# arpitbansal297/Cold-Diffusion-Models

Hardware: AMD Instinct MI355X
Metric: unet_train_imgs_per_sec (higher is better)
Workload: dtype f32 storage/accumulate; dense-conv GEMM operands bf16x3; 1 GPU; CelebA-128 denoising cold diffusion (BASELINE config 3): Unet(dim=64,(1,2,4,8),ch=3) @128x128, T=200, optimizer step = 2 micro-batches x 32 img (one fused forward / backward pass over all of them: same draws, same gradient sum) + Adam + EMA/10; per_gpu_batch=32, gradient_accumulate_every=2, parallelism=single

## Files before the change

cold-diffusion-models_amd/csrc/cdf_epilogue.h:

```cpp
#pragma once
#include "cdf_common.h"

static inline int cdf_epi_vec_ok(int Cout, const float* y, int ldy, const float* bias, const float* sbias, int ld_sbias, const float* res,
                                 int ldr, const float* pre, int ldp, const float* mul, int ldm) {
    const uintptr_t ptrs = (uintptr_t)y | (uintptr_t)bias | (uintptr_t)sbias | (uintptr_t)res | (uintptr_t)pre | (uintptr_t)mul;
    const int pitches = ldy | (sbias ? ld_sbias : 0) | (res ? ldr : 0) | (pre ? ldp : 0) | (mul ? ldm : 0);
    return (Cout % 4 == 0 && (ptrs & 15) == 0 && (pitches & 3) == 0) ? 1 : 0;
}

__device__ __forceinline__ void cdf_ld4(float* v, const float* p, int n, bool vec) {
    if (vec) {
        const float4 t = *(const float4*)p;
        v[0] = t.x; v[1] = t.y; v[2] = t.z; v[3] = t.w;
    } else {
#pragma unroll
        for (int e = 0; e < 4; ++e) v[e] = e < n ? p[e] : 0.f;
    }
}

__device__ __forceinline__ void cdf_st4(float* p, const float* v, int n, bool vec) {
    if (vec) {
        *(float4*)p = make_float4(v[0], v[1], v[2], v[3]);
    } else {
#pragma unroll
        for (int e = 0; e < 4; ++e)
            if (e < n) p[e] = v[e];
    }
}

template <int BN, int RP, int NTHR = 256, class Args, class Phase, class RowMap>
__device__ __forceinline__ void cdf_epilogue_rows(const Args& a, const Phase& ph, float* Y, const float* cs, int m_base, int n_base, int M,
                                                  int tid, RowMap rowmap, long long pix_off = 0) {
    constexpr int CP = BN + 8, TPR = BN / 4, RPS = NTHR / TPR;
    const int c4 = (tid % TPR) * 4, co = n_base + c4;
    if (co >= a.Cout) return;
    const int nval = a.Cout - co < 4 ? a.Cout - co : 4;
    const bool vec = a.vec != 0;
    const bool direct = (a.os == 1 && a.QH == a.OH && a.QW == a.OW);
    const int qhw = a.QH * a.QW;
    float bv[4] = {0.f, 0.f, 0.f, 0.f};
    if (a.bias) cdf_ld4(bv, a.bias + co, nval, vec);
    long long prev = 0, o_pre = co, o_mul = co, o_res = co, o_y = co, o_ys = co;
    bool first = true;
    for (int p = tid / TPR; p < RP; p += RPS) {
        const int m = m_base + rowmap(p);
        if (m >= M) continue;
        long long opix;
        int b;
        if (direct) {
            opix = m;
            b = m / qhw;
        } else {
            const int qx = m % a.QW, t2 = m / a.QW;
            const int qy = t2 % a.QH;
            b = t2 / a.QH;
            opix = ((long long)b * a.OH + qy * a.os + ph.oy) * a.OW + qx * a.os + ph.ox;
        }
        opix += pix_off;
        if (first) {
            o_pre += opix * a.ldp; o_mul += opix * a.ldm; o_res += opix * a.ldr; o_y += opix * a.ldy; o_ys += opix * a.ld_ys;
            first = false;
        } else {
            const int d = (int)(opix - prev);
            o_pre += (long long)d * a.ldp; o_mul += (long long)d * a.ldm; o_res += (long long)d * a.ldr; o_y += (long long)d * a.ldy;
            o_ys += (long long)d * a.ld_ys;
        }
        prev = opix;
        const float4 t = *(const float4*)(cs + p * CP + c4);
        float v[4] = {t.x + bv[0], t.y + bv[1], t.z + bv[2], t.w + bv[3]};
        float u[4];
        if (a.sbias) {
            cdf_ld4(u, a.sbias + (long long)b * a.ld_sbias + co, nval, vec);
#pragma unroll
            for (int e = 0; e < 4; ++e) v[e] += u[e];
        }
        if (a.pre && (a.io_bf & CDF_IO_PRE_GRAD)) {
            float gr[4];
#pragma unroll
            for (int e = 0; e < 4; ++e) {
                if (a.act == 1) {
                    v[e] = cdf_gelu_both(v[e], gr[e]);
                } else {
                    gr[e] = cdf_silu_grad(v[e]);
                    v[e] = cdf_silu(v[e]);
                }
            }
            if (a.io_bf & CDF_IO_PRE_BF16) cdf_st4_bf(a.pre, o_pre, gr);
            else cdf_st4(a.pre + o_pre, gr, nval, vec);
        } else {
        if (a.pre) {
            if (a.io_bf & CDF_IO_PRE_BF16) cdf_st4_bf(a.pre, o_pre, v);
            else cdf_st4(a.pre + o_pre, v, nval, vec);
        }
        if (a.act == 1) {
#pragma unroll
            for (int e = 0; e < 4; ++e) v[e] = cdf_gelu(v[e]);
        } else if (a.act == 2) {
#pragma unroll
            for (int e = 0; e < 4; ++e) v[e] = cdf_silu(v[e]);
        } else if (a.act == 3) {
#pragma unroll
            for (int e = 0; e < 4; ++e) v[e] = fmaxf(v[e], 0.0f);
        }
        }
        if (a.mul_mode) {
            if (a.io_bf & CDF_IO_MUL_BF16) cdf_ld4_bf(u, a.mul, o_mul);
            else cdf_ld4(u, a.mul + o_mul, nval, vec);
#pragma unroll
            for (int e = 0; e < 4; ++e) v[e] *= (a.mul_mode == 1 ? cdf_gelu_grad(u[e]) : (a.mul_mode == 2 ? cdf_silu_grad(u[e]) : u[e]));
        }
        if (a.res) {
            if (a.io_bf & CDF_IO_RES_BF16) cdf_ld4_bf(u, a.res, o_res);
            else cdf_ld4(u, a.res + o_res, nval, vec);
#pragma unroll
            for (int e = 0; e < 4; ++e) v[e] += u[e];
        }
        if (Y) {
            float* dst = Y + o_y;
            if (a.accumulate) {
                cdf_ld4(u, dst, nval, vec);
#pragma unroll
                for (int e = 0; e < 4; ++e) v[e] += u[e];
            }
            cdf_st4(dst, v, nval, vec);
        }
        if (a.ys_hi && vec)
            cdf_split_store4(a.ys_hi + o_ys, a.ys_lo ? a.ys_lo + o_ys : nullptr, v);
    }
}

typedef unsigned cdf_u32x2 __attribute__((ext_vector_type(2)));
#ifdef CDF_EMU
#define CDF_OPAQUE_V(x) ((void)0)
#else
#define CDF_OPAQUE_V(x) asm volatile("" : "+v"(x))
#endif

template <int ACT_, int PRE_, int MUL_, bool RES_, bool ACC_, bool HASY_, int YS_, int IO_>
struct EpiSpec {
    static constexpr int ACT = ACT_, PRE = PRE_, MUL = MUL_, YS = YS_, IO = IO_;
    static constexpr bool RES = RES_, ACC = ACC_, HASY = HASY_;
};
typedef EpiSpec<0, 0, 0, false, false, true, 0, 0> EpiPlain;
typedef EpiSpec<0, 0, 0, true, false, true, 0, 0> EpiRes;
typedef EpiSpec<1, 1, 0, false, false, false, 2, 0> EpiGeluPrePlanes;
typedef EpiSpec<1, 0, 0, false, false, false, 2, 0> EpiGeluPlanes;
typedef EpiSpec<0, 0, 1, false, false, false, 2, 0> EpiMulGeluPlanes;
typedef EpiSpec<0, 0, 0, false, true, true, 0, 0> EpiAcc;
typedef EpiSpec<0, 0, 0, false, false, false, 1, 0> EpiBfPlain;
typedef EpiSpec<0, 0, 0, true, false, false, 1, CDF_IO_RES_BF16> EpiBfRes;
typedef EpiSpec<1, 1, 0, false, false, false, 1, CDF_IO_PRE_BF16> EpiBfGeluPre;
typedef EpiSpec<1, 0, 0, false, false, false, 1, 0> EpiBfGelu;
typedef EpiSpec<0, 0, 1, false, false, false, 1, CDF_IO_MUL_BF16> EpiBfMulGelu;
#define CDF_EPI_NSPEC 11

template <class Args>
static inline int cdf_epi_select(const Args& a) {
    if (!a.vec || a.os != 1 || a.QH != a.OH || a.QW != a.OW) return 0;
    const bool pre = a.pre != nullptr, mul = a.mul_mode != 0, res = a.res != nullptr, acc = a.accumulate != 0, y = a.y != nullptr;
    const int ys = a.ys_hi ? (a.ys_lo ? 2 : 1) : 0, io = a.io_bf;
    if (io & CDF_IO_PRE_GRAD) return 0;
    auto is = [&](int ACT, int PRE, int MUL, bool RES, bool ACC, bool HASY, int YS, int IO) {
        return a.act == ACT && (pre ? 1 : 0) == PRE && a.mul_mode == MUL && res == RES && acc == ACC && y == HASY && ys == YS &&
               (io & ((PRE ? CDF_IO_PRE_BF16 : 0) | (MUL ? CDF_IO_MUL_BF16 : 0) | (RES ? CDF_IO_RES_BF16 : 0))) == IO;
    };
    (void)mul;
    if (is(0, 0, 0, false, false, true, 0, 0)) return 1;
    if (is(0, 0, 0, true, false, true, 0, 0)) return 2;
    if (is(1, 1, 0, false, false, false, 2, 0)) return 3;
    if (is(1, 0, 0, false, false, false, 2, 0)) return 4;
    if (is(0, 0, 1, false, false, false, 2, 0)) return 5;
    if (is(0, 0, 0, false, true, true, 0, 0)) return 6;
    if (is(0, 0, 0, false, false, false, 1, 0)) return 7;
    if (is(0, 0, 0, true, false, false, 1, CDF_IO_RES_BF16)) return 8;
    if (is(1, 1, 0, false, false, false, 1, CDF_IO_PRE_BF16)) return 9;
    if (is(1, 0, 0, false, false, false, 1, 0)) return 10;
    if (is(0, 0, 1, false, false, false, 1, CDF_IO_MUL_BF16)) return 11;
    return 0;
}

template <int TILE_ROWS, int BN, class Args>
__device__ __forceinline__ bool cdf_epi_tile_ok(const Args& a, int M) {
    return a.epi != 0 && M % TILE_ROWS == 0 && a.Cout % BN == 0 && (a.sbias == nullptr || (a.QH * a.QW) % TILE_ROWS == 0);
}

template <bool BF>
__device__ __forceinline__ f32x4_t cdf_ld_raw4(const void* base, unsigned off) {
    if constexpr (BF) {
        const cdf_u32x2 t = *(const cdf_u32x2*)((const unsigned short*)base + off);
        f32x4_t r = {__uint_as_float(t[0]), __uint_as_float(t[1]), 0.f, 0.f};
        return r;
    } else {
        return *(const f32x4_t*)((const float*)base + off);
    }
}
template <bool BF>
__device__ __forceinline__ f32x4_t cdf_cvt_raw4(const f32x4_t& r) {
    if constexpr (BF) {
        const unsigned x = __float_as_uint(r[0]), y = __float_as_uint(r[1]);
        f32x4_t v = {__uint_as_float(x << 16), __uint_as_float(x & 0xFFFF0000u), __uint_as_float(y << 16), __uint_as_float(y & 0xFFFF0000u)};
        return v;
    } else {
        return r;
    }
}
template <bool BF>
__device__ __forceinline__ void cdf_st_raw4(void* base, unsigned off, const f32x4_t& v) {
    if constexpr (BF) {
        cdf_u32x2 h;
        h[0] = cdf_pack2bf(v[0], v[1]);
        h[1] = cdf_pack2bf(v[2], v[3]);
        *(cdf_u32x2*)((unsigned short*)base + off) = h;
    } else {
        *(f32x4_t*)((float*)base + off) = v;
    }
}

template <int BN, int NTHR, class Args>
__device__ __forceinline__ void cdf_epi_load_bias(const Args& a, f32x4_t (&bs)[2], long long row0, int n_base, int tid) {
    int c4 = (tid % (BN / 4)) * 4;
    CDF_OPAQUE_V(c4);
    const int co = n_base + c4;
    const long long b = a.sbias ? row0 / (a.QH * a.QW) : 0;
    const float* pb = a.bias ? a.bias + co : (const float*)cdf_zero_page;
    const float* ps = a.sbias ? a.sbias + b * a.ld_sbias + co : (const float*)cdf_zero_page;
    bs[0] = *(const f32x4_t*)pb;
    bs[1] = *(const f32x4_t*)ps;
}

template <int BN, int RP, int NTHR, class S>
struct cdf_epi_fast {
    static constexpr int CP = BN + 8, TPR = BN / 4, RPS = NTHR / TPR, NR = RP / RPS;
    static_assert(NR >= 1 && NR * RPS == RP, "rows of a pass must divide among the threads");
    static_assert((S::RES ? 1 : 0) + (S::MUL ? 1 : 0) + (S::ACC ? 1 : 0) <= 1, "one loaded operand per row");
    static constexpr bool RES_BF = (S::IO & CDF_IO_RES_BF16) != 0, MUL_BF = (S::IO & CDF_IO_MUL_BF16) != 0, PRE_BF = (S::IO & CDF_IO_PRE_BF16) != 0;
    template <class Args>
    __device__ __forceinline__ static f32x4_t load_row(const Args& a, long long row0, int co, int p0, int k) {
        if constexpr (S::RES) {
            const void* base = RES_BF ? (const void*)((const unsigned short*)a.res + row0 * a.ldr) : (const void*)((const float*)a.res + row0 * a.ldr);
            return cdf_ld_raw4<RES_BF>(base, (unsigned)(p0 + k * RPS) * (unsigned)a.ldr + (unsigned)co);
        } else if constexpr (S::MUL != 0) {
            const void* base = MUL_BF ? (const void*)((const unsigned short*)a.mul + row0 * a.ldm) : (const void*)((const float*)a.mul + row0 * a.ldm);
            return cdf_ld_raw4<MUL_BF>(base, (unsigned)(p0 + k * RPS) * (unsigned)a.ldm + (unsigned)co);
        } else {
            return *(const f32x4_t*)(a.y + row0 * a.ldy + (unsigned)(p0 + k * RPS) * (unsigned)a.ldy + (unsigned)co);
        }
    }
    static constexpr bool LOADS = S::RES || S::MUL != 0 || S::ACC;
    template <class Args>
    __device__ __forceinline__ static void load(const Args& a, f32x4_t (&q)[NR], long long row0, int n_base, int tid) {
        if constexpr (LOADS) {
            int c4 = (tid % TPR) * 4, p0 = tid / TPR;
            CDF_OPAQUE_V(c4);
            CDF_OPAQUE_V(p0);
            const int co = n_base + c4;
#pragma unroll
            for (int k = 0; k < NR; ++k) q[k] = load_row(a, row0, co, p0, k);
        }
    }
    template <bool NEXT = false, class Args>
    __device__ __forceinline__ static void finish(const Args& a, f32x4_t (&q)[NR], const f32x4_t (&bs)[2], const float* cs, long long row0, int n_base, int tid,
                                                  long long next_row0 = 0) {
        int c4 = (tid % TPR) * 4, p0 = tid / TPR;
        CDF_OPAQUE_V(c4);
        CDF_OPAQUE_V(p0);
        const int co = n_base + c4;
        finish_rows<NEXT>(a, q, cs, row0, co, c4, p0, bs[0], bs[1], a.sbias != nullptr, next_row0);
    }
    template <bool NEXT, class Args>
    __device__ __forceinline__ static void finish_rows(const Args& a, f32x4_t (&q)[NR], const float* cs, long long row0, int co, int c4, int p0,
                                                       const f32x4_t& bv, const f32x4_t& sb, const bool has_sb, long long next_row0) {
        float* const ybase = S::HASY ? a.y + row0 * a.ldy : nullptr;
        void* const pbase = S::PRE ? (PRE_BF ? (void*)((unsigned short*)a.pre + row0 * a.ldp) : (void*)((float*)a.pre + row0 * a.ldp)) : nullptr;
        unsigned short* const hbase = S::YS ? a.ys_hi + row0 * a.ld_ys : nullptr;
        unsigned short* const lbase = S::YS == 2 ? a.ys_lo + row0 * a.ld_ys : nullptr;
        f32x4_t nxt = *(const f32x4_t*)(cs + (unsigned)p0 * CP + c4);
#pragma unroll
        for (int k = 0; k < NR; ++k) {
            const unsigned p = (unsigned)(p0 + k * RPS);
            f32x4_t v = nxt;
            if (k + 1 < NR) nxt = *(const f32x4_t*)(cs + (p + RPS) * CP + c4);
#pragma unroll
            for (int e = 0; e < 4; ++e) v[e] += bv[e];
            if (has_sb) {
#pragma unroll
                for (int e = 0; e < 4; ++e) v[e] += sb[e];
            }
            if constexpr (S::PRE == 1) cdf_st_raw4<PRE_BF>(pbase, p * (unsigned)a.ldp + (unsigned)co, v);
            if constexpr (S::ACT == 1) {
#pragma unroll
                for (int e = 0; e < 4; ++e) v[e] = cdf_gelu(v[e]);
            } else if constexpr (S::ACT == 2) {
#pragma unroll
                for (int e = 0; e < 4; ++e) v[e] = cdf_silu(v[e]);
            }
            if constexpr (S::MUL != 0) {
                const f32x4_t u = cdf_cvt_raw4<MUL_BF>(q[k]);
#pragma unroll
                for (int e = 0; e < 4; ++e) v[e] *= (S::MUL == 1 ? cdf_gelu_grad(u[e]) : (S::MUL == 2 ? cdf_silu_grad(u[e]) : u[e]));
            }
            if constexpr (S::RES) {
                const f32x4_t u = cdf_cvt_raw4<RES_BF>(q[k]);
#pragma unroll
                for (int e = 0; e < 4; ++e) v[e] += u[e];
            }
            if constexpr (S::ACC) {
#pragma unroll
                for (int e = 0; e < 4; ++e) v[e] += q[k][e];
            }
            if constexpr (NEXT && LOADS) q[k] = load_row(a, next_row0, co, p0, k);
            if constexpr (S::HASY) *(f32x4_t*)(ybase + p * (unsigned)a.ldy + (unsigned)co) = v;
            if constexpr (S::YS != 0) {
                uint2 h, l;
                cdf_split4(v[0], v[1], v[2], v[3], h, l);
                const unsigned o = p * (unsigned)a.ld_ys + (unsigned)co;
                *(uint2*)(hbase + o) = h;
                if constexpr (S::YS == 2) *(uint2*)(lbase + o) = l;
            }
            CDF_SCHED_FENCE();
        }
    }
};

template <bool BF_FAMILY, class F>
__device__ __forceinline__ void cdf_epi_dispatch(int id, F&& f) {
    if constexpr (!BF_FAMILY) {
        switch (id) {
            case 1: f(EpiPlain{}); break;
            case 2: f(EpiRes{}); break;
            case 3: f(EpiGeluPrePlanes{}); break;
            case 4: f(EpiGeluPlanes{}); break;
            case 5: f(EpiMulGeluPlanes{}); break;
            default: f(EpiAcc{}); break;
        }
    } else {
        switch (id) {
            case 7: f(EpiBfPlain{}); break;
            case 8: f(EpiBfRes{}); break;
            case 9: f(EpiBfGeluPre{}); break;
            case 10: f(EpiBfGelu{}); break;
            default: f(EpiBfMulGelu{}); break;
        }
    }
}
__device__ __forceinline__ bool cdf_epi_family_ok(int id, bool bf_family) { return bf_family ? (id >= 7 && id <= 11) : (id >= 1 && id <= 6); }


#define CDF_EPI_LNBWD 12
template <int BM, int BN, int NTHR, class Args, class Dump>
__device__ __forceinline__ void cdf_epi_lnbwd(const Args& a, float* cs, int tile_m, int tid, Dump&& dump) {
    constexpr int CP = BN + 8, TPR = BN / 4, RPS = NTHR / TPR, NR = BM / RPS;
    static_assert(NR >= 1 && NR * RPS == BM && (TPR & (TPR - 1)) == 0 && TPR <= 64, "rows divide among the threads; a row is a power-of-two lane group");
    int c4 = (tid % TPR) * 4, p0 = tid / TPR;
    CDF_OPAQUE_V(c4);
    CDF_OPAQUE_V(p0);
    const long long row0 = (long long)tile_m * BM;
    const f32x4_t g = *(const f32x4_t*)(a.bias + c4);
    const float* xb = a.ln_x + row0 * a.ld_lnx;
    const float* mb = a.ln_mean + row0;
    const float* rb = a.ln_rstd + row0;
    f32x4_t x[NR];
    float mean[NR], rstd[NR];
#pragma unroll
    for (int k = 0; k < NR; ++k) {
        const unsigned r = (unsigned)(p0 + k * RPS);
        x[k] = *(const f32x4_t*)(xb + r * (unsigned)a.ld_lnx + (unsigned)c4);
        mean[k] = mb[r];
        rstd[k] = rb[r];
    }
    dump();
    CDF_LDS_BARRIER();
    float* const ybase = a.y + row0 * a.ldy;
    const float inv_c = 1.0f / (float)BN;
    f32x4_t dg = {0.f, 0.f, 0.f, 0.f}, db = {0.f, 0.f, 0.f, 0.f};
    f32x4_t nxt = *(const f32x4_t*)(cs + (unsigned)p0 * CP + c4);
#pragma unroll
    for (int k = 0; k < NR; ++k) {
        const unsigned p = (unsigned)(p0 + k * RPS);
        const f32x4_t d = nxt;
        if (k + 1 < NR) nxt = *(const f32x4_t*)(cs + (p + RPS) * CP + c4);
        f32x4_t xh, gy, o;
#pragma unroll
        for (int e = 0; e < 4; ++e) {
            xh[e] = (x[k][e] - mean[k]) * rstd[k];
            dg[e] += d[e] * xh[e];
            db[e] += d[e];
            gy[e] = d[e] * g[e];
        }
        float s1 = (gy[0] + gy[1]) + (gy[2] + gy[3]);
        float s2 = (gy[0] * xh[0] + gy[1] * xh[1]) + (gy[2] * xh[2] + gy[3] * xh[3]);
        s1 = cdf_group_sum(s1, TPR) * inv_c;
        s2 = cdf_group_sum(s2, TPR) * inv_c;
#pragma unroll
        for (int e = 0; e < 4; ++e) o[e] = rstd[k] * (gy[e] - s1 - xh[e] * s2);
        *(f32x4_t*)(ybase + p * (unsigned)a.ldy + (unsigned)c4) = o;
        CDF_SCHED_FENCE();
    }
    CDF_LDS_BARRIER();
    float* red = cs;
    *(f32x4_t*)(red + ((unsigned)p0 * 2 + 0) * BN + c4) = dg;
    *(f32x4_t*)(red + ((unsigned)p0 * 2 + 1) * BN + c4) = db;
    CDF_LDS_BARRIER();
    for (int e = tid; e < 2 * BN; e += NTHR) {
        float t = 0.f;
#pragma unroll 4
        for (int r = 0; r < RPS; ++r) t += red[r * 2 * BN + e];
        a.ln_part[(long long)tile_m * 2 * BN + e] = t;
    }
}
```

cold-diffusion-models_amd/csrc/k_conv_rowhalo.hip:

```cpp
#include "cdf_conv_sp.h"

template <int W, int BN, int NS = 3, int NCH = 2, int BM = 256>
__global__ void __launch_bounds__(512, 1) conv_igemm_rowhalo_stream_kernel(SpxArgs a) {
    constexpr int WM = BM / 64, WN = 8 / WM, NW = 8, BK = 32, RE = 32, MT = BM / WM / 32, NB = 3;
    static_assert(BM == 256 && WM * WN == 8 && MT == 2, "8 waves (4 x 2) of 64-row tiles");
    static_assert(NCH % 2 == 0, "an even number of tap-row groups per tile returns the pipeline to row buffer 0");
    constexpr int EROWS = BM / 2;
    constexpr int TH = BM / W, HW2 = W + 2, RH = TH * HW2;
    constexpr int NSEG = (RH + 15) / 16, HRP = NSEG * 16;
    constexpr int TAG = (NSEG + NW - 1) / NW;
    constexpr int NT = BN / WN / 32;
    constexpr int SB = BN / 16 / NW;
    static_assert(SB * NW * 16 == BN || BN == 64, "B tile must split into 16-row segments");
    constexpr int SBI = BN == 64 ? 1 : SB;
    constexpr int PLANE_A = HRP * RE, ABUF = 2 * PLANE_A;
    constexpr int PLANE_B = BN * RE, BSTAGE = 2 * PLANE_B;
    constexpr int OFF_A1 = ABUF + 2 * BSTAGE, OFF_B2 = OFF_A1 + ABUF;
    CDF_DYN_SMEM(smem_raw);
    unsigned short* smem = (unsigned short*)smem_raw;
    float* const cs = (float*)(smem + OFF_A1);
    constexpr int CP = BN + 8;
    static_assert((size_t)OFF_A1 * 2 + (size_t)EROWS * CP * 4 <= 160 * 1024, "the staging tile must fit behind the live operand buffers");

    const int tid = threadIdx.x, lane = tid & 63, wave = __builtin_amdgcn_readfirstlane(tid >> 6);
    const int wm = wave / WN, wn = wave % WN;
    const int M = a.B * a.QH * a.QW;
    const int tiles_n = (a.Cout + BN - 1) / BN, tiles_m = M / BM, ntiles = tiles_m * tiles_n;
    const SpPhase& ph = a.ph[0];
    const int tpi = a.H / TH;

    const int srow = lane >> 2;
    const int q8 = ((lane & 3) ^ ((lane >> 4) & 3)) * 8;
    int a_seg[TAG], a_ry[TAG], a_x[TAG];
#pragma unroll
    for (int q = 0; q < TAG; ++q) {
        int g = wave + NW * q;
        if (g >= NSEG) g -= (g / NSEG) * NSEG;
        a_seg[q] = g;
        const int r = g * 16 + srow;
        a_ry[q] = r < RH ? r / HW2 : -(1 << 20);
        a_x[q] = r - (r / HW2) * HW2 - 1;
    }
    auto fetch_a = [&](int img, int y0, int c, int dy, int buf) {
        unsigned short* base = smem + (buf ? OFF_A1 : 0);
#pragma unroll
        for (int q = 0; q < TAG; ++q) {
            const int y = y0 + a_ry[q] + dy;
            const bool ok = img >= 0 && (unsigned)y < (unsigned)a.H && (unsigned)a_x[q] < (unsigned)W;
            const size_t off = ((size_t)(((ok ? img : 0) * a.H + (ok ? y : 0)) * W + (ok ? a_x[q] : 0))) * (unsigned)a.ldx + (unsigned)(c * BK + q8);
            unsigned short* seg = base + a_seg[q] * 16 * RE;
            CDF_GLDS16_K(ok ? a.x_hi + off : a.zero, seg);
            if constexpr (NS == 3) CDF_GLDS16_K(ok ? a.x_lo + off : a.zero, seg + PLANE_A);
        }
    };
    auto fetch_b = [&](int tile_n, int c, int wi, int stage) {
        unsigned short* st = smem + (stage == 2 ? OFF_B2 : ABUF + stage * BSTAGE);
#pragma unroll
        for (int p = 0; p < SBI; ++p) {
            const int seg = BN == 64 ? (wave & 3) : wave * SB + p;
            const int n = tile_n * BN + seg * 16 + srow;
            const int brow = n < a.Cout ? n : a.Cout - 1;
            const size_t woff = (size_t)((unsigned)wi * (unsigned)a.Cout + (unsigned)brow) * (unsigned)a.ldk + (unsigned)(c * BK + q8);
            CDF_GLDS16_K(a.w_hi + woff, st + seg * 16 * RE);
            if constexpr (NS == 3) CDF_GLDS16_K(a.w_lo + woff, st + PLANE_B + seg * 16 * RE);
        }
    };
    constexpr int NPL = NS == 3 ? 2 : 1;
    constexpr int PB = NPL * SBI, PAG = NPL * TAG;

    const int half = lane >> 5, l31 = lane & 31;
    int row0[MT];
#pragma unroll
    for (int i = 0; i < MT; ++i) {
        const int pix = wm * (BM / WM) + i * 32 + l31;
        const int py = pix / W, px = pix - py * W;
        row0[i] = py * HW2 + px + 1;
    }
    const bool late = a.dephase != 0 && wave >= NW / 2;

    auto tile_pos = [&](int v, int& img, int& y0, int& tn, int& tm) {
        if (v < ntiles) {
            const int tile = cdf_sp_swizzle(v, ntiles);
            tm = tile / tiles_n;
            tn = tile - tm * tiles_n;
            img = tm / tpi;
            y0 = (tm - img * tpi) * TH;
        } else {
            img = -1; y0 = 0; tn = 0; tm = 0;
        }
    };
    int img, y0, tile_n, tile_m;
    int v = blockIdx.x;
    tile_pos(v, img, y0, tile_n, tile_m);
    const bool fast_epi = cdf_epi_tile_ok<BM, BN>(a, M) && cdf_epi_family_ok(a.epi, NS == 1);
    fetch_a(img, y0, 0, ph.dy[0], 0);
    fetch_b(tile_n, 0, ph.wi[0], 0);
    fetch_b(tile_n, 0, ph.wi[1], 1);
    CDF_WAIT_DMA_LEAVE(PB);
    CDF_LDS_BARRIER();

    while (img >= 0) {
        int img_n, y0_n, tile_n_n, tile_m_n;
        tile_pos(v + gridDim.x, img_n, y0_n, tile_n_n, tile_m_n);
        f32x16_t acc[MT][NT];
#pragma unroll
        for (int i = 0; i < MT; ++i)
#pragma unroll
            for (int j = 0; j < NT; ++j)
#pragma unroll
                for (int r = 0; r < 16; ++r) acc[i][j][r] = 0.f;
        bf16x8_v ah[2][MT], al[2][MT], bh[2][NT], bl[2][NT];
        if (late) {
#pragma unroll
            for (int ks = 0; ks < 2; ++ks) {
#pragma unroll
                for (int i = 0; i < MT; ++i)
#pragma unroll
                    for (int e = 0; e < 8; ++e) { ah[ks][i][e] = 0; al[ks][i][e] = 0; }
#pragma unroll
                for (int j = 0; j < NT; ++j)
#pragma unroll
                    for (int e = 0; e < 8; ++e) { bh[ks][j][e] = 0; bl[ks][j][e] = 0; }
            }
        }
        auto mma_frags = [&]() { cdf_mma_tile<NS, MT, NT>(acc, ah, al, bh, bl); };
        int row0t[MT], l31t = l31;
#pragma unroll
        for (int i = 0; i < MT; ++i) row0t[i] = row0[i];
#ifndef CDF_EMU
#pragma unroll
        for (int i = 0; i < MT; ++i) asm volatile("" : "+v"(row0t[i]));
        asm volatile("" : "+v"(l31t));
#endif
        const int swbt = (l31t >> 2) & 3;
#pragma unroll
        for (int g = 0; g < 3; ++g) {
#pragma unroll
            for (int c = 0; c < NCH; ++c) {
#pragma unroll
                for (int i3 = 0; i3 < 3; ++i3) {
                    const int t = 3 * g + i3;
                    const int step = (g * NCH + c) * 3 + i3;
                    const int par = (g * NCH + c) & 1, rd = step % NB;
                    {
                        const int s2 = step + 2, gc2 = (s2 / 3) % (3 * NCH);
                        const bool over = s2 >= 9 * NCH;
                        const int g2 = gc2 / NCH, c2 = gc2 - g2 * NCH;
                        fetch_b(over ? tile_n_n : tile_n, c2, ph.wi[3 * g2 + s2 % 3], s2 % NB);
                    }
                    if (i3 == 0) {
                        const bool lastc = c + 1 == NCH, over = lastc && g == 2;
                        const int nc = lastc ? 0 : c + 1, ng = over ? 0 : (lastc ? g + 1 : g);
                        fetch_a(over ? img_n : img, over ? y0_n : y0, nc, ph.dy[3 * ng], par ^ 1);
                    }
                    int sa_e = par ? OFF_A1 : 0, sb_e = rd == 2 ? OFF_B2 : ABUF + rd * BSTAGE;
#ifndef CDF_EMU
                    asm volatile("" : "+s"(sa_e), "+s"(sb_e));
#endif
                    const unsigned short* sa = smem + sa_e;
                    const unsigned short* sb = smem + sb_e;
                    const int dx = ph.dx[t];
                    auto read_frags = [&]() {
#pragma unroll
                        for (int ks = 0; ks < 2; ++ks) {
#pragma unroll
                            for (int i = 0; i < MT; ++i) {
                                const int row = row0t[i] + dx;
                                const int off = row * RE + ((ks * 2 + half) ^ ((row >> 2) & 3)) * 8;
                                ah[ks][i] = *(const bf16x8_v*)(sa + off);
                                if constexpr (NS == 3) al[ks][i] = *(const bf16x8_v*)(sa + PLANE_A + off);
                            }
                            const int kc = ((ks * 2 + half) ^ swbt) * 8;
#pragma unroll
                            for (int j = 0; j < NT; ++j) {
                                const int offb = (wn * (BN / WN) + j * 32 + l31t) * RE + kc;
                                bh[ks][j] = *(const bf16x8_v*)(sb + offb);
                                if constexpr (NS == 3) bl[ks][j] = *(const bf16x8_v*)(sb + PLANE_B + offb);
                            }
                        }
                    };
                    if (late) {
                        mma_frags();
                        CDF_SCHED_FENCE();
                    }
                    read_frags();
                    if (!late) mma_frags();
                    if (i3 <= 1)
                        CDF_WAIT_DMA_LEAVE(PB + PAG);
                    else
                        CDF_WAIT_DMA_LEAVE(PB);
                    CDF_LDS_BARRIER();
                }
            }
        }
        if (late) mma_frags();
        auto dump = [&](int hp) {
            if ((wm * 64) / EROWS == hp) {
                int base = (wm * 64 - hp * EROWS + 4 * half) * CP + wn * (BN / WN) + l31;
#ifndef CDF_EMU
                asm volatile("" : "+v"(base));
#endif
                float* cb = cs + base;
#pragma unroll
                for (int i = 0; i < MT; ++i)
#pragma unroll
                    for (int j = 0; j < NT; ++j)
#pragma unroll
                        for (int r = 0; r < 16; ++r)
                            cb[(i * 32 + (r & 3) + 8 * (r >> 2)) * CP + j * 32] = acc[i][j][r];
            }
        };
        if (fast_epi) {
            const long long trow = (long long)tile_m * BM;
            cdf_epi_dispatch<NS == 1>(a.epi, [&](auto spec) {
                using E = cdf_epi_fast<BN, EROWS, 512, decltype(spec)>;
                f32x4_t q[E::NR], bs[2];
                cdf_epi_load_bias<BN, 512>(a, bs, trow, tile_n * BN, tid);
                E::load(a, q, trow, tile_n * BN, tid);
                dump(0);
                CDF_LDS_BARRIER();
                E::template finish<true>(a, q, bs, cs, trow, tile_n * BN, tid, trow + EROWS);
                CDF_LDS_BARRIER();
                dump(1);
                CDF_LDS_BARRIER();
                E::template finish<false>(a, q, bs, cs, trow + EROWS, tile_n * BN, tid);
                CDF_LDS_BARRIER();
            });
        } else {
#pragma unroll 1
            for (int hp = 0; hp < 2; ++hp) {
                dump(hp);
                CDF_LDS_BARRIER();
                cdf_epilogue_rows<BN, EROWS, 512>(a, ph, a.y, cs, tile_m * BM + hp * EROWS, tile_n * BN, M, tid, [](int p) { return p; });
                CDF_LDS_BARRIER();
            }
        }
        img = img_n; y0 = y0_n; tile_n = tile_n_n; tile_m = tile_m_n;
        v += gridDim.x;
    }
    CDF_WAIT_DMA_LEAVE(0);
}

template <int NS, int W, int BN>
static int launch_igemm_rowhalo_stream(const SpxArgs& a, int M, hipStream_t s, int reserve, CdfPlan* plan) {
    constexpr int TH = 256 / W, RH = TH * (W + 2), HRP = (RH + 15) / 16 * 16;
    constexpr size_t st_a = (size_t)2 * HRP * 64, st_b = (size_t)2 * BN * 64;
    constexpr size_t lds_s = (st_a + 2 * st_b) + ((st_a + st_b) > (size_t)128 * (BN + 8) * 4 ? (st_a + st_b) : (size_t)128 * (BN + 8) * 4);
    static_assert(lds_s <= 160 * 1024, "streaming row-halo tile does not fit the LDS");
#ifndef CDF_EMU
    static CdfDeviceLatch attr_done;
    if (!plan && attr_done.first()) {
        (void)hipFuncSetAttribute((const void*)conv_igemm_rowhalo_stream_kernel<W, BN, NS, 2>, hipFuncAttributeMaxDynamicSharedMemorySize, 160 * 1024);
        (void)hipFuncSetAttribute((const void*)conv_igemm_rowhalo_stream_kernel<W, BN, NS, 4>, hipFuncAttributeMaxDynamicSharedMemorySize, 160 * 1024);
    }
#endif
    const int tiles = (M / 256) * cdf_cdiv(a.Cout, BN);
#ifdef CDF_EMU
    int ncu = cdf_num_cus() - reserve;
    if (ncu < 1) ncu = 1;
#else
    int ncu = cdf_num_cus() - (reserve + 7) / 8 * 8;
    if (ncu < 8) ncu = 8;
#endif
    const int grid = tiles < ncu ? tiles : ncu;
    if (plan) return cdf_plan_set(plan, CDF_FORM_ROWHALO, 256, BN, a.Cin == 64 ? 2 : 4, 1, W, tiles, grid);
    if (a.Cin == 64)
        CDF_LAUNCH((conv_igemm_rowhalo_stream_kernel<W, BN, NS, 2>), dim3(grid), dim3(512), lds_s, s, a);
    else
        CDF_LAUNCH((conv_igemm_rowhalo_stream_kernel<W, BN, NS, 4>), dim3(grid), dim3(512), lds_s, s, a);
    return cdf_check_launch("conv_igemm_rowhalo_stream");
}


template <int NS>
static int launch_rowhalo_ns(int W, bool n64, const SpxArgs& a, int M, hipStream_t s, int reserve, CdfPlan* plan) {
#define CDF_ROWHALO_CASE(WW) \
    if (W == WW) return n64 ? launch_igemm_rowhalo_stream<NS, WW, 64>(a, M, s, reserve, plan) : launch_igemm_rowhalo_stream<NS, WW, 128>(a, M, s, reserve, plan);
    CDF_ROWHALO_CASE(128)
#ifdef CDF_EMU
    CDF_ROWHALO_CASE(64) CDF_ROWHALO_CASE(32) CDF_ROWHALO_CASE(16)
#endif
#undef CDF_ROWHALO_CASE
    return CDF_E_UNSUPPORTED;
}

int cdf_launch_igemm_rowhalo(int ns, int W, bool n64, const SpxArgs& a, int M, hipStream_t s, int reserve, CdfPlan* plan) {
    return ns == 3 ? launch_rowhalo_ns<3>(W, n64, a, M, s, reserve, plan) : launch_rowhalo_ns<1>(W, n64, a, M, s, reserve, plan);
}
```

Baseline: 1237 img/s.

## Restructure row-halo conv kernel to 4 waves with quarter-tile staged epilogue

Moves the streaming row-halo implicit-GEMM conv from 8 waves of 64-row tiles to 4 waves of 128-row tiles, doubling per-wave accumulator tiles and fragment reuse. The staging tile gets its own dedicated LDS region and the epilogue now runs in four 64-row quarters. The main loop is fully unrolled at compile time and gains scaffolding to interleave the previous tile's epilogue rows with MFMA groups through sched_group_barrier. That overlap path is disabled by a hard-coded false, so only the wave and tile restructuring and the quarter epilogue run. The 'late' dephase path is removed. The change risks higher register pressure, fewer waves to hide latency, and more epilogue barriers.

```diff
diff --git a/cold-diffusion-models_amd/csrc/cdf_epilogue.h b/cold-diffusion-models_amd/csrc/cdf_epilogue.h
--- a/cold-diffusion-models_amd/csrc/cdf_epilogue.h
+++ b/cold-diffusion-models_amd/csrc/cdf_epilogue.h
@@ -280,45 +280,71 @@
             const unsigned p = (unsigned)(p0 + k * RPS);
             f32x4_t v = nxt;
             if (k + 1 < NR) nxt = *(const f32x4_t*)(cs + (p + RPS) * CP + c4);
-#pragma unroll
-            for (int e = 0; e < 4; ++e) v[e] += bv[e];
-            if (has_sb) {
-#pragma unroll
-                for (int e = 0; e < 4; ++e) v[e] += sb[e];
-            }
-            if constexpr (S::PRE == 1) cdf_st_raw4<PRE_BF>(pbase, p * (unsigned)a.ldp + (unsigned)co, v);
-            if constexpr (S::ACT == 1) {
-#pragma unroll
-                for (int e = 0; e < 4; ++e) v[e] = cdf_gelu(v[e]);
-            } else if constexpr (S::ACT == 2) {
-#pragma unroll
-                for (int e = 0; e < 4; ++e) v[e] = cdf_silu(v[e]);
-            }
-            if constexpr (S::MUL != 0) {
-                const f32x4_t u = cdf_cvt_raw4<MUL_BF>(q[k]);
-#pragma unroll
-                for (int e = 0; e < 4; ++e) v[e] *= (S::MUL == 1 ? cdf_gelu_grad(u[e]) : (S::MUL == 2 ? cdf_silu_grad(u[e]) : u[e]));
-            }
-            if constexpr (S::RES) {
-                const f32x4_t u = cdf_cvt_raw4<RES_BF>(q[k]);
-#pragma unroll
-                for (int e = 0; e < 4; ++e) v[e] += u[e];
-            }
-            if constexpr (S::ACC) {
-#pragma unroll
-                for (int e = 0; e < 4; ++e) v[e] += q[k][e];
-            }
+            row_value(a, v, q[k], pbase, p, co, bv, sb, has_sb);
             if constexpr (NEXT && LOADS) q[k] = load_row(a, next_row0, co, p0, k);
-            if constexpr (S::HASY) *(f32x4_t*)(ybase + p * (unsigned)a.ldy + (unsigned)co) = v;
-            if constexpr (S::YS != 0) {
-                uint2 h, l;
-                cdf_split4(v[0], v[1], v[2], v[3], h, l);
-                const unsigned o = p * (unsigned)a.ld_ys + (unsigned)co;
-                *(uint2*)(hbase + o) = h;
-                if constexpr (S::YS == 2) *(uint2*)(lbase + o) = l;
-            }
+            row_out(a, v, ybase, hbase, lbase, p, co);
             CDF_SCHED_FENCE();
         }
+    }
+    template <class Args>
+    __device__ __forceinline__ static void row_value(const Args& a, f32x4_t& v, const f32x4_t& qk, void* pbase, unsigned p, int co, const f32x4_t& bv,
+                                                     const f32x4_t& sb, const bool has_sb) {
+#pragma unroll
+        for (int e = 0; e < 4; ++e) v[e] += bv[e];
+        if (has_sb) {
+#pragma unroll
+            for (int e = 0; e < 4; ++e) v[e] += sb[e];
+        }
+        if constexpr (S::PRE == 1) cdf_st_raw4<PRE_BF>(pbase, p * (unsigned)a.ldp + (unsigned)co, v);
+        if constexpr (S::ACT == 1) {
+#pragma unroll
+            for (int e = 0; e < 4; ++e) v[e] = cdf_gelu(v[e]);
+        } else if constexpr (S::ACT == 2) {
+#pragma unroll
+            for (int e = 0; e < 4; ++e) v[e] = cdf_silu(v[e]);
+        }
+        if constexpr (S::MUL != 0) {
+            const f32x4_t u = cdf_cvt_raw4<MUL_BF>(qk);
+#pragma unroll
+            for (int e = 0; e < 4; ++e) v[e] *= (S::MUL == 1 ? cdf_gelu_grad(u[e]) : (S::MUL == 2 ? cdf_silu_grad(u[e]) : u[e]));
+        }
+        if constexpr (S::RES) {
+            const f32x4_t u = cdf_cvt_raw4<RES_BF>(qk);
+#pragma unroll
+            for (int e = 0; e < 4; ++e) v[e] += u[e];
+        }
+        if constexpr (S::ACC) {
+#pragma unroll
+            for (int e = 0; e < 4; ++e) v[e] += qk[e];
+        }
+    }
+    template <class Args>
+    __device__ __forceinline__ static void row_out(const Args& a, const f32x4_t& v, float* ybase, unsigned short* hbase, unsigned short* lbase, unsigned p,
+                                                   int co) {
+        if constexpr (S::HASY) *(f32x4_t*)(ybase + p * (unsigned)a.ldy + (unsigned)co) = v;
+        if constexpr (S::YS != 0) {
+            uint2 h, l;
+            cdf_split4(v[0], v[1], v[2], v[3], h, l);
+            const unsigned o = p * (unsigned)a.ld_ys + (unsigned)co;
+            *(uint2*)(hbase + o) = h;
+            if constexpr (S::YS == 2) *(uint2*)(lbase + o) = l;
+        }
+    }
+    template <class Args>
+    __device__ __forceinline__ static void one_row(const Args& a, const f32x4_t (&q)[NR], const f32x4_t (&bs)[2], const float* cs, long long row0,
+                                                   int n_base, int tid, int k) {
+        int c4 = (tid % TPR) * 4, p0 = tid / TPR;
+        CDF_OPAQUE_V(c4);
+        CDF_OPAQUE_V(p0);
+        const int co = n_base + c4;
+        float* const ybase = S::HASY ? a.y + row0 * a.ldy : nullptr;
+        void* const pbase = S::PRE ? (PRE_BF ? (void*)((unsigned short*)a.pre + row0 * a.ldp) : (void*)((float*)a.pre + row0 * a.ldp)) : nullptr;
+        unsigned short* const hbase = S::YS ? a.ys_hi + row0 * a.ld_ys : nullptr;
+        unsigned short* const lbase = S::YS == 2 ? a.ys_lo + row0 * a.ld_ys : nullptr;
+        const unsigned p = (unsigned)(p0 + k * RPS);
+        f32x4_t v = *(const f32x4_t*)(cs + p * CP + c4);
+        row_value(a, v, q[k], pbase, p, co, bs[0], bs[1], a.sbias != nullptr);
+        row_out(a, v, ybase, hbase, lbase, p, co);
     }
 };
 
diff --git a/cold-diffusion-models_amd/csrc/k_conv_rowhalo.hip b/cold-diffusion-models_amd/csrc/k_conv_rowhalo.hip
--- a/cold-diffusion-models_amd/csrc/k_conv_rowhalo.hip
+++ b/cold-diffusion-models_amd/csrc/k_conv_rowhalo.hip
@@ -1,26 +1,92 @@
 #include "cdf_conv_sp.h"
 
+#include <utility>
+template <class F, int... I>
+__device__ __forceinline__ void cdf_static_for_impl(F&& f, std::integer_sequence<int, I...>) {
+    (f(std::integral_constant<int, I>{}), ...);
+}
+template <int N, class F>
+__device__ __forceinline__ void cdf_static_for(F&& f) {
+    cdf_static_for_impl(f, std::make_integer_sequence<int, N>{});
+}
+
+#ifdef CDF_EMU
+#define CDF_SCHED_GROUP(mask, n) ((void)0)
+#else
+#define CDF_SCHED_GROUP(mask, n) __builtin_amdgcn_sched_group_barrier(mask, n, 0)
+#endif
+
+template <int I0, int MT, int NT, int CP>
+__device__ __forceinline__ void cdf_rowhalo_dump2(const f32x16_t (&A)[MT][NT], float* cb) {
+#pragma unroll
+    for (int i = 0; i < 2; ++i)
+#pragma unroll
+        for (int j = 0; j < NT; ++j) {
+#pragma unroll
+            for (int r = 0; r < 16; ++r) cb[(i * 32 + (r & 3) + 8 * (r >> 2)) * CP + j * 32] = A[I0 + i][j][r];
+            CDF_SCHED_FENCE();
+        }
+}
+
+template <int NRQ, int NG>
+struct cdf_rowhalo_rows {
+    static constexpr int step(int k) { return k * 3 / NRQ; }
+    static constexpr int first(int rs) {
+        int k = 0;
+        while (k < NRQ && step(k) != rs) ++k;
+        return k;
+    }
+    static constexpr int count(int rs) {
+        int n = 0;
+        for (int k = 0; k < NRQ; ++k) n += step(k) == rs ? 1 : 0;
+        return n;
+    }
+    static constexpr int group(int k) { return (k - first(step(k))) * NG / count(step(k)); }
+    static constexpr bool here(int k, int rs, int gi) { return step(k) == rs && group(k) == gi; }
+    static constexpr bool any(int rs, int gi) {
+        for (int k = 0; k < NRQ; ++k)
+            if (here(k, rs, gi)) return true;
+        return false;
+    }
+    static constexpr int max_per_group() {
+        int m = 0;
+        for (int rs = 0; rs < 3; ++rs)
+            for (int gi = 0; gi < NG; ++gi) {
+                int n = 0;
+                for (int k = 0; k < NRQ; ++k) n += here(k, rs, gi) ? 1 : 0;
+                m = n > m ? n : m;
+            }
+        return m;
+    }
+};
+
 template <int W, int BN, int NS = 3, int NCH = 2, int BM = 256>
-__global__ void __launch_bounds__(512, 1) conv_igemm_rowhalo_stream_kernel(SpxArgs a) {
-    constexpr int WM = BM / 64, WN = 8 / WM, NW = 8, BK = 32, RE = 32, MT = BM / WM / 32, NB = 3;
-    static_assert(BM == 256 && WM * WN == 8 && MT == 2, "8 waves (4 x 2) of 64-row tiles");
+__global__ void __launch_bounds__(256, 1) conv_igemm_rowhalo_stream_kernel(SpxArgs a) {
+    constexpr int WM = 2, WN = 2, NW = 4, NTHR = 64 * NW, BK = 32, RE = 32, MT = BM / WM / 32, NB = 3;
+    static_assert(BM == 256 && MT == 4, "4 waves (2 x 2) of 128-row tiles");
     static_assert(NCH % 2 == 0, "an even number of tap-row groups per tile returns the pipeline to row buffer 0");
-    constexpr int EROWS = BM / 2;
+    constexpr int QROWS = 64, NQ = BM / QROWS;
     constexpr int TH = BM / W, HW2 = W + 2, RH = TH * HW2;
     constexpr int NSEG = (RH + 15) / 16, HRP = NSEG * 16;
     constexpr int TAG = (NSEG + NW - 1) / NW;
     constexpr int NT = BN / WN / 32;
     constexpr int SB = BN / 16 / NW;
-    static_assert(SB * NW * 16 == BN || BN == 64, "B tile must split into 16-row segments");
-    constexpr int SBI = BN == 64 ? 1 : SB;
+    static_assert(SB * NW * 16 == BN, "B tile must split into 16-row segments");
     constexpr int PLANE_A = HRP * RE, ABUF = 2 * PLANE_A;
     constexpr int PLANE_B = BN * RE, BSTAGE = 2 * PLANE_B;
-    constexpr int OFF_A1 = ABUF + 2 * BSTAGE, OFF_B2 = OFF_A1 + ABUF;
+    constexpr int OFF_A1 = ABUF + 2 * BSTAGE, OFF_B2 = OFF_A1 + ABUF, OFF_CS = OFF_B2 + BSTAGE;
     CDF_DYN_SMEM(smem_raw);
     unsigned short* smem = (unsigned short*)smem_raw;
-    float* const cs = (float*)(smem + OFF_A1);
+    float* const cs = (float*)(smem + OFF_CS);
     constexpr int CP = BN + 8;
-    static_assert((size_t)OFF_A1 * 2 + (size_t)EROWS * CP * 4 <= 160 * 1024, "the staging tile must fit behind the live operand buffers");
+    static_assert((size_t)OFF_CS * 2 + (size_t)QROWS * CP * 4 <= 160 * 1024, "operand buffers + staging tile must fit the LDS");
+    constexpr int NSTEP = 9 * NCH, SQ = NSTEP / NQ;
+    static_assert(SQ >= 4 && (NQ - 1) * SQ + 4 < NSTEP, "a quarter needs the steps d SQ .. d SQ + 4, its staging tile d SQ + 1 .. d SQ + 4");
+    constexpr int TPR = BN / 4, RPS = NTHR / TPR, NRQ = QROWS / RPS;
+    constexpr int NG = NS == 3 ? 6 : 2;
+    using RowAt = cdf_rowhalo_rows<NRQ, NG>;
+    static_assert(NRQ >= 3, "three row steps per quarter");
+    constexpr int RPG = RowAt::max_per_group();
 
     const int tid = threadIdx.x, lane = tid & 63, wave = __builtin_amdgcn_readfirstlane(tid >> 6);
     const int wm = wave / WN, wn = wave % WN;
@@ -56,8 +122,8 @@
     auto fetch_b = [&](int tile_n, int c, int wi, int stage) {
         unsigned short* st = smem + (stage == 2 ? OFF_B2 : ABUF + stage * BSTAGE);
 #pragma unroll
-        for (int p = 0; p < SBI; ++p) {
-            const int seg = BN == 64 ? (wave & 3) : wave * SB + p;
+        for (int p = 0; p < SB; ++p) {
+            const int seg = wave * SB + p;
             const int n = tile_n * BN + seg * 16 + srow;
             const int brow = n < a.Cout ? n : a.Cout - 1;
             const size_t woff = (size_t)((unsigned)wi * (unsigned)a.Cout + (unsigned)brow) * (unsigned)a.ldk + (unsigned)(c * BK + q8);
@@ -66,7 +132,8 @@
         }
     };
     constexpr int NPL = NS == 3 ? 2 : 1;
-    constexpr int PB = NPL * SBI, PAG = NPL * TAG;
+    constexpr int PB = NPL * SB, PAG = NPL * TAG;
+    static_assert(3 * PB + PAG + NRQ + 2 + 3 * NRQ <= 63, "DMA + a slice's loads and stores in flight must fit the 6-bit vmcnt");
 
     const int half = lane >> 5, l31 = lane & 31;
     int row0[MT];
@@ -76,7 +143,6 @@
         const int py = pix / W, px = pix - py * W;
         row0[i] = py * HW2 + px + 1;
     }
-    const bool late = a.dephase != 0 && wave >= NW / 2;
 
     auto tile_pos = [&](int v, int& img, int& y0, int& tn, int& tm) {
         if (v < ntiles) {
@@ -87,6 +153,16 @@
             y0 = (tm - img * tpi) * TH;
         } else {
             img = -1; y0 = 0; tn = 0; tm = 0;
+        }
+    };
+    auto dump_q = [&](const f32x16_t (&A)[MT][NT], int qd) {
+        if (wm == (qd >> 1)) {
+            int base = (4 * half) * CP + wn * (BN / WN) + l31;
+#ifndef CDF_EMU
+            asm volatile("" : "+v"(base));
+#endif
+            if (qd & 1) cdf_rowhalo_dump2<2, MT, NT, CP>(A, cs + base);
+            else cdf_rowhalo_dump2<0, MT, NT, CP>(A, cs + base);
         }
     };
     int img, y0, tile_n, tile_m;
@@ -99,6 +175,11 @@
     CDF_WAIT_DMA_LEAVE(PB);
     CDF_LDS_BARRIER();
 
+    f32x16_t prev[MT][NT];
+    f32x4_t pq[NRQ], pbs[2];
+    bool pend = false;
+    long long p_row = 0;
+    int p_n = 0;
     while (img >= 0) {
         int img_n, y0_n, tile_n_n, tile_m_n;
         tile_pos(v + gridDim.x, img_n, y0_n, tile_n_n, tile_m_n);
@@ -109,21 +190,21 @@
             for (int j = 0; j < NT; ++j)
 #pragma unroll
                 for (int r = 0; r < 16; ++r) acc[i][j][r] = 0.f;
-        bf16x8_v ah[2][MT], al[2][MT], bh[2][NT], bl[2][NT];
-        if (late) {
-#pragma unroll
-            for (int ks = 0; ks < 2; ++ks) {
-#pragma unroll
-                for (int i = 0; i < MT; ++i)
-#pragma unroll
-                    for (int e = 0; e < 8; ++e) { ah[ks][i][e] = 0; al[ks][i][e] = 0; }
-#pragma unroll
-                for (int j = 0; j < NT; ++j)
-#pragma unroll
-                    for (int e = 0; e < 8; ++e) { bh[ks][j][e] = 0; bl[ks][j][e] = 0; }
-            }
-        }
-        auto mma_frags = [&]() { cdf_mma_tile<NS, MT, NT>(acc, ah, al, bh, bl); };
+        bf16x8_v ah[MT], al[MT], bh[NT], bl[NT];
+        auto mma_group = [&](int term) {
+#pragma unroll
+            for (int i = 0; i < MT; ++i)
+#pragma unroll
+                for (int j = 0; j < NT; ++j) {
+                    if constexpr (NS == 3) {
+                        if (term == 0) acc[i][j] = CDF_MFMA_BF16(al[i], bh[j], acc[i][j]);
+                        else if (term == 1) acc[i][j] = CDF_MFMA_BF16(ah[i], bl[j], acc[i][j]);
+                        else acc[i][j] = CDF_MFMA_BF16(ah[i], bh[j], acc[i][j]);
+                    } else {
+                        acc[i][j] = CDF_MFMA_BF16(ah[i], bh[j], acc[i][j]);
+                    }
+                }
+        };
         int row0t[MT], l31t = l31;
 #pragma unroll
         for (int i = 0; i < MT; ++i) row0t[i] = row0[i];
@@ -133,105 +214,123 @@
         asm volatile("" : "+v"(l31t));
 #endif
         const int swbt = (l31t >> 2) & 3;
-#pragma unroll
-        for (int g = 0; g < 3; ++g) {
-#pragma unroll
-            for (int c = 0; c < NCH; ++c) {
-#pragma unroll
-                for (int i3 = 0; i3 < 3; ++i3) {
-                    const int t = 3 * g + i3;
-                    const int step = (g * NCH + c) * 3 + i3;
-                    const int par = (g * NCH + c) & 1, rd = step % NB;
-                    {
-                        const int s2 = step + 2, gc2 = (s2 / 3) % (3 * NCH);
-                        const bool over = s2 >= 9 * NCH;
-                        const int g2 = gc2 / NCH, c2 = gc2 - g2 * NCH;
-                        fetch_b(over ? tile_n_n : tile_n, c2, ph.wi[3 * g2 + s2 % 3], s2 % NB);
+        cdf_static_for<NSTEP>([&](auto STEP) {
+            constexpr int step = decltype(STEP)::value;
+            constexpr int gc = step / 3, i3 = step % 3, g = gc / NCH, c = gc % NCH;
+            constexpr int t = 3 * g + i3;
+            constexpr int par = gc & 1, rd = step % NB;
+            constexpr int qd = step / SQ, sp = step % SQ;
+            if constexpr (qd < NQ && sp == 1) {
+                if (pend) {
+                    cdf_epi_dispatch<NS == 1>(a.epi, [&](auto spec) {
+                        using E = cdf_epi_fast<BN, QROWS, NTHR, decltype(spec)>;
+                        if constexpr (qd == 0) cdf_epi_load_bias<BN, NTHR>(a, pbs, p_row, p_n, tid);
+                        E::load(a, pq, p_row + qd * QROWS, p_n, tid);
+                    });
+                    dump_q(prev, qd);
+                }
+            }
+            {
+                constexpr int s2 = step + 2, gc2 = (s2 / 3) % (3 * NCH);
+                constexpr bool over = s2 >= 9 * NCH;
+                constexpr int g2 = gc2 / NCH, c2 = gc2 - g2 * NCH;
+                fetch_b(over ? tile_n_n : tile_n, c2, ph.wi[3 * g2 + s2 % 3], s2 % NB);
+            }
+            if constexpr (i3 == 0) {
+                constexpr bool lastc = c + 1 == NCH, over = lastc && g == 2;
+                constexpr int nc = lastc ? 0 : c + 1, ng = over ? 0 : (lastc ? g + 1 : g);
+                fetch_a(over ? img_n : img, over ? y0_n : y0, nc, ph.dy[3 * ng], par ^ 1);
+            }
+            int sa_e = par ? OFF_A1 : 0, sb_e = rd == 2 ? OFF_B2 : ABUF + rd * BSTAGE;
+#ifndef CDF_EMU
+            asm volatile("" : "+s"(sa_e), "+s"(sb_e));
+#endif
+            const unsigned short* sa = smem + sa_e;
+            const unsigned short* sb = smem + sb_e;
+            const int dx = ph.dx[t];
+            constexpr int rq = step >= 2 ? (step - 2) / SQ : NQ, rs = step - 2 - rq * SQ;
+            constexpr bool row_step = rq < NQ && rs < 3;
+            cdf_static_for<2>([&](auto KS) {
+                constexpr int ks = decltype(KS)::value;
+#pragma unroll
+                for (int i = 0; i < MT; ++i) {
+                    const int row = row0t[i] + dx;
+                    const int off = row * RE + ((ks * 2 + half) ^ ((row >> 2) & 3)) * 8;
+                    ah[i] = *(const bf16x8_v*)(sa + off);
+                    if constexpr (NS == 3) al[i] = *(const bf16x8_v*)(sa + PLANE_A + off);
+                }
+                const int kc = ((ks * 2 + half) ^ swbt) * 8;
+#pragma unroll
+                for (int j = 0; j < NT; ++j) {
+                    const int offb = (wn * (BN / WN) + j * 32 + l31t) * RE + kc;
+                    bh[j] = *(const bf16x8_v*)(sb + offb);
+                    if constexpr (NS == 3) bl[j] = *(const bf16x8_v*)(sb + PLANE_B + offb);
+                }
+                cdf_static_for<NG / 2>([&](auto TERM) {
+                    constexpr int term = decltype(TERM)::value, gi = ks * (NG / 2) + term;
+                    if constexpr (row_step && RowAt::any(row_step ? rs : 0, gi)) {
+                        if (pend) {
+                            cdf_epi_dispatch<NS == 1>(a.epi, [&](auto spec) {
+                                using E = cdf_epi_fast<BN, QROWS, NTHR, decltype(spec)>;
+                                mma_group(term);
+                                cdf_static_for<NRQ>([&](auto K) {
+                                    constexpr int k = decltype(K)::value;
+                                    if constexpr (RowAt::here(k, rs, gi)) E::one_row(a, pq, pbs, cs, p_row + rq * QROWS, p_n, tid, k);
+                                });
+#pragma unroll
+                                for (int m = 0; m < MT * NT; ++m) {
+                                    CDF_SCHED_GROUP(0x008, 1);
+                                    CDF_SCHED_GROUP(0x002 | 0x004 | 0x010 | 0x080, 6 * RPG);
+                                }
+                            });
+                        } else {
+                            mma_group(term);
+                        }
+                    } else {
+                        mma_group(term);
                     }
-                    if (i3 == 0) {
-                        const bool lastc = c + 1 == NCH, over = lastc && g == 2;
-                        const int nc = lastc ? 0 : c + 1, ng = over ? 0 : (lastc ? g + 1 : g);
-                        fetch_a(over ? img_n : img, over ? y0_n : y0, nc, ph.dy[3 * ng], par ^ 1);
-                    }
-                    int sa_e = par ? OFF_A1 : 0, sb_e = rd == 2 ? OFF_B2 : ABUF + rd * BSTAGE;
-#ifndef CDF_EMU
-                    asm volatile("" : "+s"(sa_e), "+s"(sb_e));
-#endif
-                    const unsigned short* sa = smem + sa_e;
-                    const unsigned short* sb = smem + sb_e;
-                    const int dx = ph.dx[t];
-                    auto read_frags = [&]() {
-#pragma unroll
-                        for (int ks = 0; ks < 2; ++ks) {
-#pragma unroll
-                            for (int i = 0; i < MT; ++i) {
-                                const int row = row0t[i] + dx;
-                                const int off = row * RE + ((ks * 2 + half) ^ ((row >> 2) & 3)) * 8;
-                                ah[ks][i] = *(const bf16x8_v*)(sa + off);
-                                if constexpr (NS == 3) al[ks][i] = *(const bf16x8_v*)(sa + PLANE_A + off);
-                            }
-                            const int kc = ((ks * 2 + half) ^ swbt) * 8;
-#pragma unroll
-                            for (int j = 0; j < NT; ++j) {
-                                const int offb = (wn * (BN / WN) + j * 32 + l31t) * RE + kc;
-                                bh[ks][j] = *(const bf16x8_v*)(sb + offb);
-                                if constexpr (NS == 3) bl[ks][j] = *(const bf16x8_v*)(sb + PLANE_B + offb);
-                            }
-                        }
-                    };
-                    if (late) {
-                        mma_frags();
-                        CDF_SCHED_FENCE();
-                    }
-                    read_frags();
-                    if (!late) mma_frags();
-                    if (i3 <= 1)
-                        CDF_WAIT_DMA_LEAVE(PB + PAG);
-                    else
-                        CDF_WAIT_DMA_LEAVE(PB);
+                });
+            });
+            if constexpr (i3 <= 1)
+                CDF_WAIT_DMA_LEAVE(PB + PAG);
+            else
+                CDF_WAIT_DMA_LEAVE(PB);
+            CDF_LDS_BARRIER();
+        });
+        const long long trow = (long long)tile_m * BM;
+        if (fast_epi && img_n >= 0 && false) {
+#pragma unroll
+            for (int i = 0; i < MT; ++i)
+#pragma unroll
+                for (int j = 0; j < NT; ++j) {
+                    prev[i][j] = acc[i][j];
+                    CDF_SCHED_FENCE();
+                }
+            pend = true;
+            p_row = trow;
+            p_n = tile_n * BN;
+        } else if (fast_epi) {
+            pend = false;
+            cdf_epi_dispatch<NS == 1>(a.epi, [&](auto spec) {
+                using E = cdf_epi_fast<BN, QROWS, NTHR, decltype(spec)>;
+                f32x4_t q[E::NR], bs[2];
+                cdf_epi_load_bias<BN, NTHR>(a, bs, trow, tile_n * BN, tid);
+                E::load(a, q, trow, tile_n * BN, tid);
+#pragma unroll 1
+                for (int d = 0; d < NQ; ++d) {
+                    dump_q(acc, d);
                     CDF_LDS_BARRIER();
-                }
-            }
-        }
-        if (late) mma_frags();
-        auto dump = [&](int hp) {
-            if ((wm * 64) / EROWS == hp) {
-                int base = (wm * 64 - hp * EROWS + 4 * half) * CP + wn * (BN / WN) + l31;
-#ifndef CDF_EMU
-                asm volatile("" : "+v"(base));
-#endif
-                float* cb = cs + base;
-#pragma unroll
-                for (int i = 0; i < MT; ++i)
-#pragma unroll
-                    for (int j = 0; j < NT; ++j)
-#pragma unroll
-                        for (int r = 0; r < 16; ++r)
-                            cb[(i * 32 + (r & 3) + 8 * (r >> 2)) * CP + j * 32] = acc[i][j][r];
-            }
-        };
-        if (fast_epi) {
-            const long long trow = (long long)tile_m * BM;
-            cdf_epi_dispatch<NS == 1>(a.epi, [&](auto spec) {
-                using E = cdf_epi_fast<BN, EROWS, 512, decltype(spec)>;
-                f32x4_t q[E::NR], bs[2];
-                cdf_epi_load_bias<BN, 512>(a, bs, trow, tile_n * BN, tid);
-                E::load(a, q, trow, tile_n * BN, tid);
-                dump(0);
-                CDF_LDS_BARRIER();
-                E::template finish<true>(a, q, bs, cs, trow, tile_n * BN, tid, trow + EROWS);
-                CDF_LDS_BARRIER();
-                dump(1);
-                CDF_LDS_BARRIER();
-                E::template finish<false>(a, q, bs, cs, trow + EROWS, tile_n * BN, tid);
-                CDF_LDS_BARRIER();
+                    if (d + 1 < NQ) E::template finish<true>(a, q, bs, cs, trow + d * QROWS, tile_n * BN, tid, trow + (d + 1) * QROWS);
+                    else E::template finish<false>(a, q, bs, cs, trow + d * QROWS, tile_n * BN, tid);
+                    CDF_LDS_BARRIER();
+                }
             });
         } else {
 #pragma unroll 1
-            for (int hp = 0; hp < 2; ++hp) {
-                dump(hp);
+            for (int d = 0; d < NQ; ++d) {
+                dump_q(acc, d);
                 CDF_LDS_BARRIER();
-                cdf_epilogue_rows<BN, EROWS, 512>(a, ph, a.y, cs, tile_m * BM + hp * EROWS, tile_n * BN, M, tid, [](int p) { return p; });
+                cdf_epilogue_rows<BN, QROWS, NTHR>(a, ph, a.y, cs, tile_m * BM + d * QROWS, tile_n * BN, M, tid, [](int p) { return p; });
                 CDF_LDS_BARRIER();
             }
         }
@@ -245,7 +344,7 @@
 static int launch_igemm_rowhalo_stream(const SpxArgs& a, int M, hipStream_t s, int reserve, CdfPlan* plan) {
     constexpr int TH = 256 / W, RH = TH * (W + 2), HRP = (RH + 15) / 16 * 16;
     constexpr size_t st_a = (size_t)2 * HRP * 64, st_b = (size_t)2 * BN * 64;
-    constexpr size_t lds_s = (st_a + 2 * st_b) + ((st_a + st_b) > (size_t)128 * (BN + 8) * 4 ? (st_a + st_b) : (size_t)128 * (BN + 8) * 4);
+    constexpr size_t lds_s = 2 * st_a + 3 * st_b + (size_t)64 * (BN + 8) * 4;
     static_assert(lds_s <= 160 * 1024, "streaming row-halo tile does not fit the LDS");
 #ifndef CDF_EMU
     static CdfDeviceLatch attr_done;
@@ -265,9 +364,9 @@
     const int grid = tiles < ncu ? tiles : ncu;
     if (plan) return cdf_plan_set(plan, CDF_FORM_ROWHALO, 256, BN, a.Cin == 64 ? 2 : 4, 1, W, tiles, grid);
     if (a.Cin == 64)
-        CDF_LAUNCH((conv_igemm_rowhalo_stream_kernel<W, BN, NS, 2>), dim3(grid), dim3(512), lds_s, s, a);
+        CDF_LAUNCH((conv_igemm_rowhalo_stream_kernel<W, BN, NS, 2>), dim3(grid), dim3(256), lds_s, s, a);
     else
-        CDF_LAUNCH((conv_igemm_rowhalo_stream_kernel<W, BN, NS, 4>), dim3(grid), dim3(512), lds_s, s, a);
+        CDF_LAUNCH((conv_igemm_rowhalo_stream_kernel<W, BN, NS, 4>), dim3(grid), dim3(256), lds_s, s, a);
     return cdf_check_launch("conv_igemm_rowhalo_stream");
 }
 
```

After: 1226 img/s, median of 2. About the same (-0.9%).
